# ucas-vg/PointTinyBenchmark

Hardware: NVIDIA H100
Metric: cpr_head_refine_img_per_s_1333x800 (higher is better)
Workload: dtype fp32

## Files before the change

pointtinybenchmark_b200/csrc/conv_tc.cu:

```cuda
#include "tc_ptx.cuh"
#include <cuda_bf16.h>
#include <stdlib.h>
#include <type_traits>

namespace ptb {

constexpr int CV_N = 256;
constexpr int CV_N_MAX = 512;
constexpr int CV_BM = 128;
constexpr int CV_NT = 128;
constexpr int CV_KB = 16;
constexpr int CV_KB_F16 = 32;
constexpr int CV_KH = 3;
constexpr int CV_A_STAGES = 4;
constexpr int CV_B_STAGES = 8;
constexpr uint32_t CV_A_BYTES = (CV_BM + 2 * 32) * 64;
constexpr uint32_t CV_B_BYTES = CV_NT * 64;
constexpr uint32_t CV_A_STAGE_BYTES = 2 * CV_A_BYTES;
constexpr uint32_t CV_B_STAGE_BYTES = 2 * CV_B_BYTES;
constexpr uint32_t CV_RING_BYTES = CV_A_STAGES * CV_A_STAGE_BYTES + CV_B_STAGES * CV_B_STAGE_BYTES;
constexpr uint32_t CV_SMEM_BYTES = CV_RING_BYTES + 1024  + 256 ;
static_assert(CV_SMEM_BYTES <= 227 * 1024, "the conv rings must fit the 227 KB of opt-in shared memory");
static_assert(2 * 8 * (CV_A_STAGES + CV_B_STAGES) + 8 <= 256, "the conv barriers and the item counter must fit their 256 B");
constexpr int CV_THREADS = 384;

struct ConvShape {
  int B, H, W, Cin;
  int tiles_h, tiles_w;
  int n_main, n_right, n_bottom, per_img, n_tiles;
  int right_w0, right_h;
  int bottom_h0;
  int n_slices;
  int taps;
  int n_out;
  int ldy;
};

struct ConvMaps {
  CUtensorMap x[3][2];
  CUtensorMap w[2];
};
struct TileAt {
  int b, h0, w0, shape, twl;
};
__device__ __forceinline__ TileAt tile_at(const ConvShape& cs, int tile) {
  TileAt t;
  t.b = tile / cs.per_img;
  const int r = tile - t.b * cs.per_img;
  if (r < cs.n_main) {
    t.shape = 0; t.twl = 4; t.h0 = (r / cs.tiles_w) * 8; t.w0 = (r % cs.tiles_w) * 16;
  } else if (r < cs.n_main + cs.n_right) {
    t.shape = 2; t.twl = 3; t.h0 = (r - cs.n_main) * 16; t.w0 = cs.right_w0;
  } else {
    t.shape = 1; t.twl = 5; t.h0 = cs.bottom_h0; t.w0 = (r - cs.n_main - cs.n_right) * 32;
  }
  return t;
}

constexpr int CV_GN_NONE = 0, CV_GN_F16 = 1, CV_GN_F32 = 2;
constexpr int CV_APPLY_WARPS = 3;
constexpr int CV_MMA_WARPS = 8;
struct GnFuse {
  const float* gamma;
  const float* beta;
  float eps;
  void* out;
  __half* out_l;
  int* overflow_flag;
  int* done;
};
constexpr uint32_t CV_CNT_OFFSET = 2 * 8 * (CV_A_STAGES + CV_B_STAGES);

__device__ __forceinline__ int ld_acquire_gpu(const int* p) {
  int v;
  asm volatile("ld.acquire.gpu.global.b32 %0, [%1];" : "=r"(v) : "l"(p) : "memory");
  return v;
}
__device__ __forceinline__ void red_release_gpu_add(int* p, int v) {
  asm volatile("red.release.gpu.global.add.s32 [%0], %1;" ::"l"(p), "r"(v) : "memory");
}
__device__ __forceinline__ int ld_acquire_cta_shared(uint32_t a) {
  int v;
  asm volatile("ld.acquire.cta.shared::cta.b32 %0, [%1];" : "=r"(v) : "r"(a) : "memory");
  return v;
}
__device__ __forceinline__ void red_release_cta_shared_add(uint32_t a, int v) {
  asm volatile("red.release.cta.shared::cta.add.s32 [%0], %1;" ::"r"(a), "r"(v) : "memory");
}
__device__ __forceinline__ void wait_count(const int* p, int target, int lane) {
  if (lane == 0) {
    uint32_t ns = 32, polls = 0;
    while (ld_acquire_gpu(p) < target) {
      __nanosleep(ns);
      if (ns < 1024) ns <<= 1;
      if (++polls > (1u << 24)) __trap();
    }
  }
  __syncwarp();
}
__device__ __forceinline__ void publish_image(uint32_t cnt, int* done_b, int item, int last, int lane) {
  if (lane == 0) {
    const int n = (last - item) / (int)gridDim.x + 1;
    const int through = (item - (int)blockIdx.x) / (int)gridDim.x + n;
    uint32_t ns = 32, polls = 0;
    while (ld_acquire_cta_shared(cnt) < through * (CV_MMA_WARPS / 2) || ld_acquire_cta_shared(cnt + 4) < through * (CV_MMA_WARPS / 2)) {
      __nanosleep(ns);
      if (ns < 1024) ns <<= 1;
      if (++polls > (1u << 24)) __trap();
    }
    red_release_gpu_add(done_b, n * CV_MMA_WARPS);
  }
  __syncwarp();
}

template <int GN>
__device__ __forceinline__ void gn_apply_item(const ConvShape& cs, const GnFuse& gf, const float* __restrict__ y,
                                              const double* __restrict__ stats, int item, int member, int team, int lane,
                                              bool& clamped) {
  const int tile = item / cs.n_slices, n0 = (item - tile * cs.n_slices) * CV_NT;
  const TileAt ta = tile_at(cs, tile);
  const int c = n0 + 4 * lane, g = c >> 3;
  const int HW = cs.H * cs.W, cpg = CV_N / 32;
  const double inv_n = 1.0 / ((double)HW * cpg);
  const double s = __ldcg(stats + ((size_t)ta.b * 32 + g) * 2), ss = __ldcg(stats + ((size_t)ta.b * 32 + g) * 2 + 1);
  const double mean = s * inv_n;
  double var = ss * inv_n - mean * mean;
  var = var < 0.0 ? 0.0 : var;
  const float rstd = (float)(1.0 / sqrt(var + (double)gf.eps));
  const float mu = (float)mean;
  const float4 ga = __ldg(reinterpret_cast<const float4*>(gf.gamma + c)), be = __ldg(reinterpret_cast<const float4*>(gf.beta + c));
  const int h_end = ta.shape == 2 ? cs.right_h : cs.H;
  const int tw_mask = (1 << ta.twl) - 1;
  const size_t img = (size_t)ta.b * HW * CV_N + c;
  const float* __restrict__ yb = y + img;
  constexpr int U = 4;
  for (int p0 = member; p0 < CV_BM; p0 += U * team) {
    float4 v[U];
    int at[U];
#pragma unroll
    for (int u = 0; u < U; ++u) {
      const int p = p0 + u * team;
      const int h = ta.h0 + (p >> ta.twl), w = ta.w0 + (p & tw_mask);
      at[u] = p < CV_BM && h < h_end && w < cs.W ? (h * cs.W + w) * CV_N : -1;
      if (at[u] >= 0) v[u] = __ldcg(reinterpret_cast<const float4*>(yb + at[u]));
    }
#pragma unroll
    for (int u = 0; u < U; ++u) {
      if (at[u] < 0) continue;
      float o[4] = {v[u].x, v[u].y, v[u].z, v[u].w};
      o[0] = fmaf((o[0] - mu) * rstd, ga.x, be.x); o[1] = fmaf((o[1] - mu) * rstd, ga.y, be.y);
      o[2] = fmaf((o[2] - mu) * rstd, ga.z, be.z); o[3] = fmaf((o[3] - mu) * rstd, ga.w, be.w);
#pragma unroll
      for (int j = 0; j < 4; ++j) o[j] = fmaxf(o[j], 0.f);
      if constexpr (GN == CV_GN_F16) {
        __align__(8) __half h[4], l[4];
#pragma unroll
        for (int j = 0; j < 4; ++j) {
          if (fabsf(o[j]) > 60000.f) { o[j] = copysignf(60000.f, o[j]); clamped = true; }
          split_h2(o[j], h[j], l[j]);
        }
        *reinterpret_cast<uint2*>(reinterpret_cast<__half*>(gf.out) + img + at[u]) = *reinterpret_cast<uint2*>(h);
        *reinterpret_cast<uint2*>(gf.out_l + img + at[u]) = *reinterpret_cast<uint2*>(l);
      } else {
        *reinterpret_cast<float4*>(reinterpret_cast<float*>(gf.out) + img + at[u]) = make_float4(o[0], o[1], o[2], o[3]);
      }
    }
  }
}

template <bool F16, int NT, bool A_LO_ZERO = false, typename OutT = float, int GN = CV_GN_NONE>
__global__ void __launch_bounds__(CV_THREADS, 1)
conv_tc_kernel(const __grid_constant__ ConvMaps mp, ConvShape cs, OutT* __restrict__ y, double* __restrict__ stats ,
               float out_scale, const float* __restrict__ dev_out_scale, const float* __restrict__ bias, GnFuse gf) {
  static_assert(F16 || NT == 128, "the TF32 mode runs 128-channel slices");
  static_assert(F16 || (!A_LO_ZERO && std::is_same<OutT, float>::value), "half-precision inputs and outputs belong to the fp16 mode");
  static_assert(GN == CV_GN_NONE || (F16 && NT == 128 && std::is_same<OutT, float>::value), "the fused GroupNorm apply runs on fp32 y, NT 128");
  constexpr int KBC = F16 ? CV_KB_F16 : CV_KB;
  extern __shared__ uint8_t smem_raw[];
  const uint32_t smem_base = (smem_u32(smem_raw) + 1023u) & ~1023u;
  const uint32_t sA_base = smem_base, sB_base = smem_base + CV_A_STAGES * CV_A_STAGE_BYTES;
  const uint32_t bar_base = smem_base + CV_RING_BYTES;
  auto full_a = [&](int s) { return bar_base + 8u * s; };
  auto empty_a = [&](int s) { return bar_base + 8u * (CV_A_STAGES + s); };
  auto full_b = [&](int s) { return bar_base + 8u * (2 * CV_A_STAGES + s); };
  auto empty_b = [&](int s) { return bar_base + 8u * (2 * CV_A_STAGES + CV_B_STAGES + s); };

  const int wg = threadIdx.x >> 7;
  const int kblocks_per_tap = cs.Cin / KBC;
  const int n_kh = cs.taps == 9 ? CV_KH : 1;
  const int n_boxes_item = (cs.taps / n_kh) * kblocks_per_tap;
  const int n_items = cs.n_tiles * cs.n_slices;

  if (threadIdx.x == 0) {
    for (int s = 0; s < CV_A_STAGES; ++s) {
      mbar_init(full_a(s), 1);
      mbar_init(empty_a(s), 8);
    }
    for (int s = 0; s < CV_B_STAGES; ++s) {
      mbar_init(full_b(s), 1);
      mbar_init(empty_b(s), 8);
    }
    if constexpr (GN != CV_GN_NONE) asm volatile("st.shared.v2.u32 [%0], {0, 0};" ::"r"(bar_base + CV_CNT_OFFSET) : "memory");
    asm volatile("fence.mbarrier_init.release.cluster;" ::: "memory");
  }
  __syncthreads();

  if (wg == 0) {
    if constexpr (GN != CV_GN_NONE) {
      regs_dealloc<72>();
      const int warp = threadIdx.x >> 5, lane = threadIdx.x & 31;
      if (warp >= 1) {
        const int items_per_img = cs.per_img * cs.n_slices;
        bool clamped = false;
        for (int item = blockIdx.x; item < n_items; item += gridDim.x) {
          const int b = item / items_per_img;
          if (b == cs.B - 1) break;
          if (warp == 1 && item - (int)gridDim.x < b * items_per_img)
            publish_image(bar_base + CV_CNT_OFFSET, gf.done + b, item, (b + 1) * items_per_img - 1, lane);
          wait_count(gf.done + b, items_per_img * CV_MMA_WARPS, lane);
          gn_apply_item<GN>(cs, gf, y, stats, item, warp - 1, CV_APPLY_WARPS, lane, clamped);
        }
        if (clamped && gf.overflow_flag) *gf.overflow_flag = 1;
      }
    } else {
      regs_dealloc<40>();
    }
    if (threadIdx.x == 0) {
      int a_st = 0, b_st = 0;
      uint32_t a_ph = 0, b_ph = 0;
      for (int item = blockIdx.x; item < n_items; item += gridDim.x) {
        const int tile = item / cs.n_slices, n0 = (item - tile * cs.n_slices) * NT;
        const TileAt ta = tile_at(cs, tile);
        const uint32_t a_bytes = (uint32_t)(CV_BM + ((n_kh - 1) << ta.twl)) * 64u;
        for (int ks = 0; ks < n_boxes_item; ++ks) {
          const int kw = cs.taps == 9 ? ks / kblocks_per_tap : 1, cblk = ks - (ks / kblocks_per_tap) * kblocks_per_tap;
          mbar_wait(empty_a(a_st), a_ph ^ 1u);
          const uint32_t sA_hi = sA_base + a_st * CV_A_STAGE_BYTES;
          mbar_expect_tx(full_a(a_st), (A_LO_ZERO ? 1 : 2) * a_bytes);
          const int aw = ta.w0 + kw - 1, ah = ta.h0 - (n_kh > 1 ? 1 : 0);
          tma_load_4d(&mp.x[ta.shape][0], full_a(a_st), sA_hi, cblk * KBC, aw, ah, ta.b);
          if constexpr (!A_LO_ZERO) tma_load_4d(&mp.x[ta.shape][1], full_a(a_st), sA_hi + CV_A_BYTES, cblk * KBC, aw, ah, ta.b);
          if (++a_st == CV_A_STAGES) { a_st = 0; a_ph ^= 1u; }
          for (int kh = 0; kh < n_kh; ++kh) {
            const int tap = cs.taps == 9 ? 3 * kh + kw : 0;
            const int kcol = tap * cs.Cin + cblk * KBC;
            mbar_wait(empty_b(b_st), b_ph ^ 1u);
            const uint32_t sB_hi = sB_base + b_st * CV_B_STAGE_BYTES;
            mbar_expect_tx(full_b(b_st), 2 * NT * 64);
            tma_load_2d(&mp.w[0], full_b(b_st), sB_hi, kcol, n0);
            tma_load_2d(&mp.w[1], full_b(b_st), sB_hi + CV_B_BYTES, kcol, n0);
            if (++b_st == CV_B_STAGES) { b_st = 0; b_ph ^= 1u; }
          }
        }
      }
    }
  } else {
    if constexpr (GN != CV_GN_NONE) regs_alloc<216>();
    else regs_alloc<232>();
    const int cw = wg - 1;
    const int t = threadIdx.x & 127, warp = t >> 5, lane = t & 31;
    const float sc = F16 ? (dev_out_scale ? __fmul_rn(out_scale, *dev_out_scale) : out_scale) : 1.f;
    float acc[NT / 2], cor[NT / 2];
    int a_st = 0, b_st = 0;
    uint32_t a_ph = 0, b_ph = 0;
    for (int item = blockIdx.x; item < n_items; item += gridDim.x) {
      const int tile = item / cs.n_slices, n0 = (item - tile * cs.n_slices) * NT;
      const TileAt ta = tile_at(cs, tile);
      const uint32_t kh_step = 64u << ta.twl;
      auto k_loop = [&](auto kh_n_) {
        constexpr int KH_N = decltype(kh_n_)::value;
        int prev_a = 0, prev_b = 0;
        for (int ks = 0; ks < n_boxes_item; ++ks) {
          mbar_wait(full_a(a_st), a_ph);
          const uint32_t sA_hi = sA_base + a_st * CV_A_STAGE_BYTES + (uint32_t)cw * (CV_BM * 64 / 2);
          const uint32_t sA_lo = sA_hi + CV_A_BYTES;
#pragma unroll
          for (int kh = 0; kh < KH_N; ++kh) {
            mbar_wait(full_b(b_st), b_ph);
            const uint32_t a_off = kh_step * kh, sB_hi = sB_base + b_st * CV_B_STAGE_BYTES, sB_lo = sB_hi + CV_B_BYTES;
            wgmma_fence();
#pragma unroll
            for (int k = 0; k < 2; ++k) {
              const uint64_t a_hi = gmma_desc(sA_hi + a_off + 32u * k, 16u, 512u, GMMA_SW64);
              const uint64_t a_lo = gmma_desc(sA_lo + a_off + 32u * k, 16u, 512u, GMMA_SW64);
              const uint64_t b_hi = gmma_desc(sB_hi + 32u * k, 16u, 512u, GMMA_SW64), b_lo = gmma_desc(sB_lo + 32u * k, 16u, 512u, GMMA_SW64);
              const uint32_t first = (ks | kh | k) != 0;
              if constexpr (F16) {
                wgmma_f16<0, 0>(acc, a_hi, b_hi, first);
                if constexpr (A_LO_ZERO) {
                  wgmma_f16<0, 0>(cor, a_hi, b_lo, first);
                } else {
                  wgmma_f16<0, 0>(cor, a_lo, b_hi, first);
                  wgmma_f16<0, 0>(cor, a_hi, b_lo, 1u);
                }
              } else {
                wgmma_tf32(acc, a_hi, b_hi, first);
                wgmma_tf32(cor, a_lo, b_hi, first);
                wgmma_tf32(cor, a_hi, b_lo, 1u);
              }
            }
            wgmma_commit();
            if ((ks | kh) != 0) {
              wgmma_wait<1>();
              if (lane == 0) {
                mbar_arrive(empty_b(prev_b));
                if (kh == 0) mbar_arrive(empty_a(prev_a));
              }
            }
            prev_b = b_st;
            if (++b_st == CV_B_STAGES) { b_st = 0; b_ph ^= 1u; }
          }
          prev_a = a_st;
          if (++a_st == CV_A_STAGES) { a_st = 0; a_ph ^= 1u; }
        }
        wgmma_wait<0>();
        if (lane == 0) { mbar_arrive(empty_b(prev_b)); mbar_arrive(empty_a(prev_a)); }
      };
      if (n_kh == CV_KH) k_loop(std::integral_constant<int, CV_KH>{});
      else k_loop(std::integral_constant<int, 1>{});

      const int h_end = ta.shape == 2 ? cs.right_h : cs.H;
      OutT* row_ptr[2];
      bool valid[2];
#pragma unroll
      for (int j = 0; j < 2; ++j) {
        const int r = 64 * cw + 16 * warp + (lane >> 2) + 8 * j;
        const int h = ta.h0 + (r >> ta.twl), w = ta.w0 + (r & ((1 << ta.twl) - 1));
        valid[j] = h < h_end && w < cs.W;
        row_ptr[j] = y + (((size_t)ta.b * cs.H + h) * cs.W + w) * cs.ldy;
      }
      float part[NT == 128 ? 32 : 1];
#pragma unroll
      for (int i = 0; i < NT / 8; ++i) {
        const int col = n0 + 8 * i + 2 * (lane & 3);
        float s = 0.f, ss = 0.f;
#pragma unroll
        for (int j = 0; j < 2; ++j) {
          float v0 = __fadd_rn(acc[4 * i + 2 * j], cor[4 * i + 2 * j]);
          float v1 = __fadd_rn(acc[4 * i + 2 * j + 1], cor[4 * i + 2 * j + 1]);
          if (F16) { v0 = __fmul_rn(v0, sc); v1 = __fmul_rn(v1, sc); }
          if (bias) {
            if (col < cs.n_out) v0 = v0 + __ldg(bias + col);
            if (col + 1 < cs.n_out) v1 = v1 + __ldg(bias + col + 1);
          }
          if (valid[j]) {
            if constexpr (std::is_same<OutT, float>::value) {
              if (col + 1 < cs.n_out) *reinterpret_cast<float2*>(row_ptr[j] + col) = make_float2(v0, v1);
              else if (col < cs.n_out) row_ptr[j][col] = v0;
            } else if constexpr (std::is_same<OutT, __half>::value) {
              if (col + 1 < cs.n_out) *reinterpret_cast<__half2*>(row_ptr[j] + col) = __halves2half2(__float2half_rn(v0), __float2half_rn(v1));
              else if (col < cs.n_out) row_ptr[j][col] = __float2half_rn(v0);
            } else {
              if (col + 1 < cs.n_out) *reinterpret_cast<__nv_bfloat162*>(row_ptr[j] + col) = __halves2bfloat162(__float2bfloat16_rn(v0), __float2bfloat16_rn(v1));
              else if (col < cs.n_out) row_ptr[j][col] = __float2bfloat16_rn(v0);
            }
            s += v0 + v1;
            ss = fmaf(v0, v0, ss);
            ss = fmaf(v1, v1, ss);
          }
        }
        if constexpr (NT == 128) { part[2 * i] = s; part[2 * i + 1] = ss; }
      }
      if constexpr (NT == 128) {
        if (stats) {
          auto level = [&](auto o_) {
            constexpr int o = decltype(o_)::value;
            const bool up = (lane & o) != 0;
#pragma unroll
            for (int i = 0; i < o; ++i) {
              const float send = up ? part[i] : part[i + o];
              const float recv = __shfl_xor_sync(0xffffffffu, send, o);
              part[i] = (up ? part[i + o] : part[i]) + recv;
            }
          };
          level(std::integral_constant<int, 16>{}); level(std::integral_constant<int, 8>{}); level(std::integral_constant<int, 4>{});
          level(std::integral_constant<int, 2>{}); level(std::integral_constant<int, 1>{});
          atomicAdd(stats + ((size_t)ta.b * 32 + (n0 >> 3) + (lane >> 1)) * 2 + (lane & 1), (double)part[0]);
        }
      }
      if constexpr (GN != CV_GN_NONE) {
        __syncwarp();
        if (lane == 0) red_release_cta_shared_add(bar_base + CV_CNT_OFFSET + 4u * cw, 1);
      }
    }
  }
  if constexpr (GN != CV_GN_NONE) {
    const int warp = threadIdx.x >> 5, lane = threadIdx.x & 31;
    if (warp >= 1) {
      const int items_per_img = cs.per_img * cs.n_slices, last0 = (cs.B - 1) * items_per_img;
      bool clamped = false;
      int item = (int)blockIdx.x;
      if (item < last0) item += (last0 - item + (int)gridDim.x - 1) / (int)gridDim.x * (int)gridDim.x;
      if (warp == 1 && item < n_items) publish_image(bar_base + CV_CNT_OFFSET, gf.done + cs.B - 1, item, n_items - 1, lane);
      for (; item < n_items; item += gridDim.x) {
        wait_count(gf.done + cs.B - 1, items_per_img * CV_MMA_WARPS, lane);
        gn_apply_item<GN>(cs, gf, y, stats, item, warp - 1, CV_APPLY_WARPS + CV_MMA_WARPS, lane, clamped);
      }
      if (clamped && gf.overflow_flag) *gf.overflow_flag = 1;
    }
  }
}

__device__ __forceinline__ float tf32_hi(float x) { return __uint_as_float(__float_as_uint(x) & 0xFFFFE000u); }

__global__ void __launch_bounds__(256)
split_tf32_kernel(const float4* __restrict__ x, long long n4, float4* __restrict__ hi, float4* __restrict__ lo) {
  for (long long i = (long long)blockIdx.x * 256 + threadIdx.x; i < n4; i += (long long)gridDim.x * 256) {
    const float4 v = __ldcs(x + i);
    float4 h = make_float4(tf32_hi(v.x), tf32_hi(v.y), tf32_hi(v.z), tf32_hi(v.w));
    hi[i] = h;
    lo[i] = make_float4(v.x - h.x, v.y - h.y, v.z - h.z, v.w - h.w);
  }
}

__global__ void __launch_bounds__(256)
gn_relu_apply_kernel(const float4* __restrict__ y, const double* __restrict__ stats, const float* __restrict__ gamma,
                     const float* __restrict__ beta, int HW, int C, int groups, float eps, int relu, long long n4,
                     float4* __restrict__ out_hi, float4* __restrict__ out_lo) {
  const int c4n = C >> 2;
  const int cpg = C / groups;
  const double inv_n = 1.0 / ((double)HW * cpg);
  for (long long i = (long long)blockIdx.x * 256 + threadIdx.x; i < n4; i += (long long)gridDim.x * 256) {
    const int c = (int)(i % c4n) * 4;
    const long long pix = i / c4n;
    const int b = (int)(pix / HW);
    const int g = c / cpg;
    const double s = stats[((size_t)b * groups + g) * 2], ss = stats[((size_t)b * groups + g) * 2 + 1];
    const double mean = s * inv_n;
    double var = ss * inv_n - mean * mean;
    var = var < 0.0 ? 0.0 : var;
    const float rstd = (float)(1.0 / sqrt(var + (double)eps));
    const float mu = (float)mean;
    const float4 v = __ldcs(y + i);
    const float4 ga = *reinterpret_cast<const float4*>(gamma + c), be = *reinterpret_cast<const float4*>(beta + c);
    float4 o;
    o.x = fmaf((v.x - mu) * rstd, ga.x, be.x);
    o.y = fmaf((v.y - mu) * rstd, ga.y, be.y);
    o.z = fmaf((v.z - mu) * rstd, ga.z, be.z);
    o.w = fmaf((v.w - mu) * rstd, ga.w, be.w);
    if (relu) { o.x = fmaxf(o.x, 0.f); o.y = fmaxf(o.y, 0.f); o.z = fmaxf(o.z, 0.f); o.w = fmaxf(o.w, 0.f); }
    if (out_lo) {
      const float4 h = make_float4(tf32_hi(o.x), tf32_hi(o.y), tf32_hi(o.z), tf32_hi(o.w));
      out_hi[i] = h;
      out_lo[i] = make_float4(o.x - h.x, o.y - h.y, o.z - h.z, o.w - h.w);
    } else {
      out_hi[i] = o;
    }
  }
}

__device__ __forceinline__ float pow2_scale_for(float amax) {
  if (!(amax > 0.f) || !isfinite(amax)) return 1.f;
  int e;
  frexpf(amax, &e);
  return ldexpf(1.f, 12 - e);
}

__device__ __forceinline__ float amax4(float m, const float4 v) {
  return fmaxf(m, fmaxf(fmaxf(fabsf(v.x), fabsf(v.y)), fmaxf(fabsf(v.z), fabsf(v.w))));
}

__global__ void __launch_bounds__(256) amax_abs_kernel(const float4* __restrict__ x, long long n4, unsigned int* __restrict__ out_bits) {
  float m = 0.f;
  const long long step = (long long)gridDim.x * 256;
  long long i = (long long)blockIdx.x * 256 + threadIdx.x;
  for (; i + 3 * step < n4; i += 4 * step) {
    const float4 v0 = x[i], v1 = x[i + step], v2 = x[i + 2 * step], v3 = x[i + 3 * step];
    m = amax4(amax4(amax4(amax4(m, v0), v1), v2), v3);
  }
  for (; i < n4; i += step) m = amax4(m, x[i]);
  m = warp_max(m);
  if ((threadIdx.x & 31) == 0) atomicMax(out_bits, __float_as_uint(m));
}

__device__ __forceinline__ void split8(const float4 a, const float4 b, float scale, uint4& ph, uint4& pl) {
  __align__(16) __half h[8], l[8];
  split_h2(a.x * scale, h[0], l[0]); split_h2(a.y * scale, h[1], l[1]);
  split_h2(a.z * scale, h[2], l[2]); split_h2(a.w * scale, h[3], l[3]);
  split_h2(b.x * scale, h[4], l[4]); split_h2(b.y * scale, h[5], l[5]);
  split_h2(b.z * scale, h[6], l[6]); split_h2(b.w * scale, h[7], l[7]);
  ph = *reinterpret_cast<uint4*>(h);
  pl = *reinterpret_cast<uint4*>(l);
}

__global__ void __launch_bounds__(256)
split_f16_kernel(const float4* __restrict__ x, long long n4, const unsigned int* __restrict__ dev_amax_bits,
                 uint2* __restrict__ hi, uint2* __restrict__ lo, float* __restrict__ inv_scale_out) {
  const float scale = dev_amax_bits ? pow2_scale_for(__uint_as_float(*dev_amax_bits)) : 1.f;
  if (inv_scale_out && blockIdx.x == 0 && threadIdx.x == 0) *inv_scale_out = 1.f / scale;
  const long long n8 = n4 >> 1;
  const long long step = (long long)gridDim.x * 256;
  uint4* hi8 = reinterpret_cast<uint4*>(hi);
  uint4* lo8 = reinterpret_cast<uint4*>(lo);
  const bool al16 = ((reinterpret_cast<uintptr_t>(hi) | reinterpret_cast<uintptr_t>(lo)) & 15) == 0;
  long long i = (long long)blockIdx.x * 256 + threadIdx.x;
  if (al16) {
    for (; i + step < n8; i += 2 * step) {
      const float4 a0 = __ldcs(x + 2 * i), a1 = __ldcs(x + 2 * i + 1);
      const float4 b0 = __ldcs(x + 2 * (i + step)), b1 = __ldcs(x + 2 * (i + step) + 1);
      uint4 ph, pl;
      split8(a0, a1, scale, ph, pl);
      hi8[i] = ph; lo8[i] = pl;
      split8(b0, b1, scale, ph, pl);
      hi8[i + step] = ph; lo8[i + step] = pl;
    }
    for (; i < n8; i += step) {
      uint4 ph, pl;
      split8(__ldcs(x + 2 * i), __ldcs(x + 2 * i + 1), scale, ph, pl);
      hi8[i] = ph; lo8[i] = pl;
    }
    i = 2 * n8 + (long long)blockIdx.x * 256 + threadIdx.x;
  }
  for (; i < n4; i += step) {
    const float4 v = __ldcs(x + i);
    __half h[4], l[4];
    split_h2(v.x * scale, h[0], l[0]); split_h2(v.y * scale, h[1], l[1]);
    split_h2(v.z * scale, h[2], l[2]); split_h2(v.w * scale, h[3], l[3]);
    hi[i] = *reinterpret_cast<uint2*>(h);
    lo[i] = *reinterpret_cast<uint2*>(l);
  }
}

__device__ __forceinline__ void bf16x8_to_f32(const uint4 v, float4& a, float4& b) {
  a = make_float4(__uint_as_float(v.x << 16), __uint_as_float(v.x & 0xFFFF0000u), __uint_as_float(v.y << 16), __uint_as_float(v.y & 0xFFFF0000u));
  b = make_float4(__uint_as_float(v.z << 16), __uint_as_float(v.z & 0xFFFF0000u), __uint_as_float(v.w << 16), __uint_as_float(v.w & 0xFFFF0000u));
}

__global__ void __launch_bounds__(256) amax_abs_bf16_kernel(const uint4* __restrict__ x, long long n8, unsigned int* __restrict__ out_bits) {
  float m = 0.f;
  const long long step = (long long)gridDim.x * 256;
  long long i = (long long)blockIdx.x * 256 + threadIdx.x;
  float4 a, b;
  for (; i + 3 * step < n8; i += 4 * step) {
    const uint4 v0 = x[i], v1 = x[i + step], v2 = x[i + 2 * step], v3 = x[i + 3 * step];
    bf16x8_to_f32(v0, a, b); m = amax4(amax4(m, a), b);
    bf16x8_to_f32(v1, a, b); m = amax4(amax4(m, a), b);
    bf16x8_to_f32(v2, a, b); m = amax4(amax4(m, a), b);
    bf16x8_to_f32(v3, a, b); m = amax4(amax4(m, a), b);
  }
  for (; i < n8; i += step) { bf16x8_to_f32(x[i], a, b); m = amax4(amax4(m, a), b); }
  m = warp_max(m);
  if ((threadIdx.x & 31) == 0) atomicMax(out_bits, __float_as_uint(m));
}

__global__ void __launch_bounds__(256)
split_f16_from_bf16_kernel(const uint4* __restrict__ x, long long n8, const unsigned int* __restrict__ dev_amax_bits,
                           uint4* __restrict__ hi, uint4* __restrict__ lo, float* __restrict__ inv_scale_out) {
  const float scale = pow2_scale_for(__uint_as_float(*dev_amax_bits));
  if (blockIdx.x == 0 && threadIdx.x == 0) *inv_scale_out = 1.f / scale;
  const long long step = (long long)gridDim.x * 256;
  long long i = (long long)blockIdx.x * 256 + threadIdx.x;
  float4 a, b;
  uint4 ph, pl;
  for (; i + step < n8; i += 2 * step) {
    const uint4 v0 = __ldcs(x + i), v1 = __ldcs(x + i + step);
    bf16x8_to_f32(v0, a, b); split8(a, b, scale, ph, pl);
    hi[i] = ph; lo[i] = pl;
    bf16x8_to_f32(v1, a, b); split8(a, b, scale, ph, pl);
    hi[i + step] = ph; lo[i + step] = pl;
  }
  for (; i < n8; i += step) {
    bf16x8_to_f32(__ldcs(x + i), a, b); split8(a, b, scale, ph, pl);
    hi[i] = ph; lo[i] = pl;
  }
}

__global__ void __launch_bounds__(256)
gn_relu_apply_f16_kernel(const float4* __restrict__ y, const double* __restrict__ stats, const float* __restrict__ gamma,
                         const float* __restrict__ beta, int HW, int C, int groups, float eps, int relu, long long n4,
                         uint2* __restrict__ out_h, uint2* __restrict__ out_l, int* __restrict__ overflow_flag) {
  const int c4n = C >> 2;
  const int cpg = C / groups;
  const double inv_n = 1.0 / ((double)HW * cpg);
  for (long long i = (long long)blockIdx.x * 256 + threadIdx.x; i < n4; i += (long long)gridDim.x * 256) {
    const int c = (int)(i % c4n) * 4;
    const long long pix = i / c4n;
    const int b = (int)(pix / HW);
    const int g = c / cpg;
    const double s = stats[((size_t)b * groups + g) * 2], ss = stats[((size_t)b * groups + g) * 2 + 1];
    const double mean = s * inv_n;
    double var = ss * inv_n - mean * mean;
    var = var < 0.0 ? 0.0 : var;
    const float rstd = (float)(1.0 / sqrt(var + (double)eps));
    const float mu = (float)mean;
    const float4 v = __ldcs(y + i);
    const float4 ga = *reinterpret_cast<const float4*>(gamma + c), be = *reinterpret_cast<const float4*>(beta + c);
    float o[4];
    o[0] = fmaf((v.x - mu) * rstd, ga.x, be.x); o[1] = fmaf((v.y - mu) * rstd, ga.y, be.y);
    o[2] = fmaf((v.z - mu) * rstd, ga.z, be.z); o[3] = fmaf((v.w - mu) * rstd, ga.w, be.w);
    __half h[4], l[4];
#pragma unroll
    for (int j = 0; j < 4; ++j) {
      if (relu) o[j] = fmaxf(o[j], 0.f);
      if (fabsf(o[j]) > 60000.f) { o[j] = copysignf(60000.f, o[j]); if (overflow_flag) *overflow_flag = 1; }
      split_h2(o[j], h[j], l[j]);
    }
    out_h[i] = *reinterpret_cast<uint2*>(h);
    out_l[i] = *reinterpret_cast<uint2*>(l);
  }
}

__global__ void __launch_bounds__(256)
gn_relu_apply_f16_v8_kernel(const float4* __restrict__ y, const double* __restrict__ stats, const float* __restrict__ gamma,
                            const float* __restrict__ beta, int HW, int C, int groups, float eps, int relu, int pix_per_cta,
                            uint4* __restrict__ out_h, uint4* __restrict__ out_l, int* __restrict__ overflow_flag) {
  const int tpp = C >> 3;
  const int ppp = 256 / tpp;
  const int c = (threadIdx.x % tpp) * 8;
  const int b = blockIdx.y;
  const int cpg = C / groups;
  const int g = c / cpg;
  const double inv_n = 1.0 / ((double)HW * cpg);
  const double s = stats[((size_t)b * groups + g) * 2], ss = stats[((size_t)b * groups + g) * 2 + 1];
  const double mean = s * inv_n;
  double var = ss * inv_n - mean * mean;
  var = var < 0.0 ? 0.0 : var;
  const float rstd = (float)(1.0 / sqrt(var + (double)eps));
// ... 460 lines not shown
```

pointtinybenchmark_b200/csrc/tc_ptx.cuh:

```cuda
#pragma once
#include "ptb_common.cuh"
#include <cuda.h>
#include <cuda_fp16.h>

namespace ptb {

__device__ __forceinline__ uint32_t smem_u32(const void* p) { return (uint32_t)__cvta_generic_to_shared(p); }

__device__ __forceinline__ void mbar_init(uint32_t bar, uint32_t count) {
  asm volatile("mbarrier.init.shared::cta.b64 [%0], %1;" ::"r"(bar), "r"(count) : "memory");
}
__device__ __forceinline__ void mbar_expect_tx(uint32_t bar, uint32_t bytes) {
  asm volatile("mbarrier.arrive.expect_tx.shared::cta.b64 _, [%0], %1;" ::"r"(bar), "r"(bytes) : "memory");
}
__device__ __forceinline__ void mbar_arrive(uint32_t bar) {
  asm volatile("mbarrier.arrive.shared::cta.b64 _, [%0];" ::"r"(bar) : "memory");
}
__device__ __forceinline__ bool mbar_try_wait(uint32_t bar, uint32_t parity) {
  uint32_t ok;
  asm volatile(
      "{\n\t.reg .pred p;\n\t"
      "mbarrier.try_wait.parity.shared::cta.b64 p, [%1], %2;\n\t"
      "selp.u32 %0, 1, 0, p;\n\t}"
      : "=r"(ok)
      : "r"(bar), "r"(parity)
      : "memory");
  return ok != 0;
}
__device__ __forceinline__ void mbar_wait(uint32_t bar, uint32_t parity) {
  uint32_t spins = 0;
  while (!mbar_try_wait(bar, parity)) {
    if (++spins > (1u << 28)) __trap();
  }
}
__device__ __forceinline__ void tma_load_4d(const CUtensorMap* tm, uint32_t bar, uint32_t dst, int c0, int c1, int c2, int c3) {
  asm volatile(
      "cp.async.bulk.tensor.4d.shared::cluster.global.mbarrier::complete_tx::bytes [%0], [%1, {%3, %4, %5, %6}], [%2];"
      ::"r"(dst), "l"(tm), "r"(bar), "r"(c0), "r"(c1), "r"(c2), "r"(c3)
      : "memory");
}
__device__ __forceinline__ void tma_load_2d(const CUtensorMap* tm, uint32_t bar, uint32_t dst, int c0, int c1) {
  asm volatile(
      "cp.async.bulk.tensor.2d.shared::cluster.global.mbarrier::complete_tx::bytes [%0], [%1, {%3, %4}], [%2];"
      ::"r"(dst), "l"(tm), "r"(bar), "r"(c0), "r"(c1)
      : "memory");
}
__device__ __forceinline__ void fence_async_smem() { asm volatile("fence.proxy.async.shared::cta;" ::: "memory"); }

constexpr uint32_t GMMA_SW128 = 1, GMMA_SW64 = 2;
__device__ __forceinline__ uint64_t gmma_desc(uint32_t smem_addr, uint32_t lbo, uint32_t sbo, uint32_t layout) {
  uint64_t d = 0;
  d |= (uint64_t)((smem_addr & 0x3FFFF) >> 4);
  d |= (uint64_t)((lbo >> 4) & 0x3FFF) << 16;
  d |= (uint64_t)((sbo >> 4) & 0x3FFF) << 32;
  d |= (uint64_t)layout << 62;
  return d;
}
__device__ __forceinline__ void wgmma_fence() { asm volatile("wgmma.fence.sync.aligned;" ::: "memory"); }
__device__ __forceinline__ void wgmma_commit() { asm volatile("wgmma.commit_group.sync.aligned;" ::: "memory"); }
template <int N>
__device__ __forceinline__ void wgmma_wait() { asm volatile("wgmma.wait_group.sync.aligned %0;" ::"n"(N) : "memory"); }
template <int R>
__device__ __forceinline__ void regs_dealloc() { asm volatile("setmaxnreg.dec.sync.aligned.u32 %0;" ::"n"(R)); }
template <int R>
__device__ __forceinline__ void regs_alloc() { asm volatile("setmaxnreg.inc.sync.aligned.u32 %0;" ::"n"(R)); }
template <int TA, int TB>
__device__ __forceinline__ void wgmma_f16(float (&d)[64], uint64_t da, uint64_t db, uint32_t scale_d) {
  asm volatile(
      "{\n\t.reg .pred p;\n\t"
      "setp.ne.b32 p, %66, 0;\n\t"
      "wgmma.mma_async.sync.aligned.m64n128k16.f32.f16.f16 "
      "{%0, %1, %2, %3, %4, %5, %6, %7, %8, %9, %10, %11, %12, %13, %14, %15,"
      " %16, %17, %18, %19, %20, %21, %22, %23, %24, %25, %26, %27, %28, %29, %30, %31,"
      " %32, %33, %34, %35, %36, %37, %38, %39, %40, %41, %42, %43, %44, %45, %46, %47,"
      " %48, %49, %50, %51, %52, %53, %54, %55, %56, %57, %58, %59, %60, %61, %62, %63}, "
      "%64, %65, p, 1, 1, %67, %68;\n\t}"
      : "+f"(d[0]), "+f"(d[1]), "+f"(d[2]), "+f"(d[3]), "+f"(d[4]), "+f"(d[5]), "+f"(d[6]), "+f"(d[7]),
        "+f"(d[8]), "+f"(d[9]), "+f"(d[10]), "+f"(d[11]), "+f"(d[12]), "+f"(d[13]), "+f"(d[14]), "+f"(d[15]),
        "+f"(d[16]), "+f"(d[17]), "+f"(d[18]), "+f"(d[19]), "+f"(d[20]), "+f"(d[21]), "+f"(d[22]), "+f"(d[23]),
        "+f"(d[24]), "+f"(d[25]), "+f"(d[26]), "+f"(d[27]), "+f"(d[28]), "+f"(d[29]), "+f"(d[30]), "+f"(d[31]),
        "+f"(d[32]), "+f"(d[33]), "+f"(d[34]), "+f"(d[35]), "+f"(d[36]), "+f"(d[37]), "+f"(d[38]), "+f"(d[39]),
        "+f"(d[40]), "+f"(d[41]), "+f"(d[42]), "+f"(d[43]), "+f"(d[44]), "+f"(d[45]), "+f"(d[46]), "+f"(d[47]),
        "+f"(d[48]), "+f"(d[49]), "+f"(d[50]), "+f"(d[51]), "+f"(d[52]), "+f"(d[53]), "+f"(d[54]), "+f"(d[55]),
        "+f"(d[56]), "+f"(d[57]), "+f"(d[58]), "+f"(d[59]), "+f"(d[60]), "+f"(d[61]), "+f"(d[62]), "+f"(d[63])
      : "l"(da), "l"(db), "r"(scale_d), "n"(TA), "n"(TB));
}

template <int TA, int TB>
__device__ __forceinline__ void wgmma_f16(float (&d)[32], uint64_t da, uint64_t db, uint32_t scale_d) {
  asm volatile(
      "{\n\t.reg .pred p;\n\t"
      "setp.ne.b32 p, %34, 0;\n\t"
      "wgmma.mma_async.sync.aligned.m64n64k16.f32.f16.f16 "
      "{%0, %1, %2, %3, %4, %5, %6, %7, %8, %9, %10, %11, %12, %13, %14, %15,"
      " %16, %17, %18, %19, %20, %21, %22, %23, %24, %25, %26, %27, %28, %29, %30, %31}, "
      "%32, %33, p, 1, 1, %35, %36;\n\t}"
      : "+f"(d[0]), "+f"(d[1]), "+f"(d[2]), "+f"(d[3]), "+f"(d[4]), "+f"(d[5]), "+f"(d[6]), "+f"(d[7]),
        "+f"(d[8]), "+f"(d[9]), "+f"(d[10]), "+f"(d[11]), "+f"(d[12]), "+f"(d[13]), "+f"(d[14]), "+f"(d[15]),
        "+f"(d[16]), "+f"(d[17]), "+f"(d[18]), "+f"(d[19]), "+f"(d[20]), "+f"(d[21]), "+f"(d[22]), "+f"(d[23]),
        "+f"(d[24]), "+f"(d[25]), "+f"(d[26]), "+f"(d[27]), "+f"(d[28]), "+f"(d[29]), "+f"(d[30]), "+f"(d[31])
      : "l"(da), "l"(db), "r"(scale_d), "n"(TA), "n"(TB));
}

template <int TA, int TB>
__device__ __forceinline__ void wgmma_f16(float (&d)[16], uint64_t da, uint64_t db, uint32_t scale_d) {
  asm volatile(
      "{\n\t.reg .pred p;\n\t"
      "setp.ne.b32 p, %18, 0;\n\t"
      "wgmma.mma_async.sync.aligned.m64n32k16.f32.f16.f16 "
      "{%0, %1, %2, %3, %4, %5, %6, %7, %8, %9, %10, %11, %12, %13, %14, %15}, "
      "%16, %17, p, 1, 1, %19, %20;\n\t}"
      : "+f"(d[0]), "+f"(d[1]), "+f"(d[2]), "+f"(d[3]), "+f"(d[4]), "+f"(d[5]), "+f"(d[6]), "+f"(d[7]),
        "+f"(d[8]), "+f"(d[9]), "+f"(d[10]), "+f"(d[11]), "+f"(d[12]), "+f"(d[13]), "+f"(d[14]), "+f"(d[15])
      : "l"(da), "l"(db), "r"(scale_d), "n"(TA), "n"(TB));
}

template <int TA, int TB>
__device__ __forceinline__ void wgmma_f16(float (&d)[8], uint64_t da, uint64_t db, uint32_t scale_d) {
  asm volatile(
      "{\n\t.reg .pred p;\n\t"
      "setp.ne.b32 p, %10, 0;\n\t"
      "wgmma.mma_async.sync.aligned.m64n16k16.f32.f16.f16 "
      "{%0, %1, %2, %3, %4, %5, %6, %7}, "
      "%8, %9, p, 1, 1, %11, %12;\n\t}"
      : "+f"(d[0]), "+f"(d[1]), "+f"(d[2]), "+f"(d[3]), "+f"(d[4]), "+f"(d[5]), "+f"(d[6]), "+f"(d[7])
      : "l"(da), "l"(db), "r"(scale_d), "n"(TA), "n"(TB));
}

__device__ __forceinline__ void wgmma_tf32(float (&d)[64], uint64_t da, uint64_t db, uint32_t scale_d) {
  asm volatile(
      "{\n\t.reg .pred p;\n\t"
      "setp.ne.b32 p, %66, 0;\n\t"
      "wgmma.mma_async.sync.aligned.m64n128k8.f32.tf32.tf32 "
      "{%0, %1, %2, %3, %4, %5, %6, %7, %8, %9, %10, %11, %12, %13, %14, %15,"
      " %16, %17, %18, %19, %20, %21, %22, %23, %24, %25, %26, %27, %28, %29, %30, %31,"
      " %32, %33, %34, %35, %36, %37, %38, %39, %40, %41, %42, %43, %44, %45, %46, %47,"
      " %48, %49, %50, %51, %52, %53, %54, %55, %56, %57, %58, %59, %60, %61, %62, %63}, "
      "%64, %65, p, 1, 1;\n\t}"
      : "+f"(d[0]), "+f"(d[1]), "+f"(d[2]), "+f"(d[3]), "+f"(d[4]), "+f"(d[5]), "+f"(d[6]), "+f"(d[7]),
        "+f"(d[8]), "+f"(d[9]), "+f"(d[10]), "+f"(d[11]), "+f"(d[12]), "+f"(d[13]), "+f"(d[14]), "+f"(d[15]),
        "+f"(d[16]), "+f"(d[17]), "+f"(d[18]), "+f"(d[19]), "+f"(d[20]), "+f"(d[21]), "+f"(d[22]), "+f"(d[23]),
        "+f"(d[24]), "+f"(d[25]), "+f"(d[26]), "+f"(d[27]), "+f"(d[28]), "+f"(d[29]), "+f"(d[30]), "+f"(d[31]),
        "+f"(d[32]), "+f"(d[33]), "+f"(d[34]), "+f"(d[35]), "+f"(d[36]), "+f"(d[37]), "+f"(d[38]), "+f"(d[39]),
        "+f"(d[40]), "+f"(d[41]), "+f"(d[42]), "+f"(d[43]), "+f"(d[44]), "+f"(d[45]), "+f"(d[46]), "+f"(d[47]),
        "+f"(d[48]), "+f"(d[49]), "+f"(d[50]), "+f"(d[51]), "+f"(d[52]), "+f"(d[53]), "+f"(d[54]), "+f"(d[55]),
        "+f"(d[56]), "+f"(d[57]), "+f"(d[58]), "+f"(d[59]), "+f"(d[60]), "+f"(d[61]), "+f"(d[62]), "+f"(d[63])
      : "l"(da), "l"(db), "r"(scale_d));
}


__device__ __forceinline__ void split_h2(float v, __half& h, __half& l) {
  h = __float2half_rn(v);
  l = __float2half_rn(v - __half2float(h));
}

typedef CUresult (*EncodeTiledFn)(CUtensorMap*, CUtensorMapDataType, cuuint32_t, void*, const cuuint64_t*, const cuuint64_t*,
                                  const cuuint32_t*, const cuuint32_t*, CUtensorMapInterleave, CUtensorMapSwizzle,
                                  CUtensorMapL2promotion, CUtensorMapFloatOOBfill);
EncodeTiledFn tc_get_encode();

}
```

Baseline: 2405.

## Feed f16 conv wgmma A-hi operand from registers via ldmatrix

In the f16 path, the high half of the A tile is now loaded into registers with ldmatrix and used by register-sourced wgmma (RS form). Previously it was read from shared memory through a descriptor for each of the two or three MMAs that use it. The register fragments are double-buffered across kh/box iterations, and the box loop is unrolled by two so the buffer index stays compile-time. The aim is to cut repeated shared-memory operand traffic for A. The cost is extra register pressure in an already heavy consumer warpgroup, plus dependence on the swizzle address math being correct.

```diff
diff --git a/pointtinybenchmark_b200/csrc/conv_tc.cu b/pointtinybenchmark_b200/csrc/conv_tc.cu
--- a/pointtinybenchmark_b200/csrc/conv_tc.cu
+++ b/pointtinybenchmark_b200/csrc/conv_tc.cu
@@ -263,6 +263,9 @@
     float acc[NT / 2], cor[NT / 2];
     int a_st = 0, b_st = 0;
     uint32_t a_ph = 0, b_ph = 0;
+    const int a_row = 16 * warp + (lane & 15);
+    const uint32_t a_lane[2] = {(uint32_t)(a_row * 64 + (((0 + (lane >> 4)) ^ ((a_row >> 1) & 3)) << 4)),
+                                (uint32_t)(a_row * 64 + (((2 + (lane >> 4)) ^ ((a_row >> 1) & 3)) << 4))};
     for (int item = blockIdx.x; item < n_items; item += gridDim.x) {
       const int tile = item / cs.n_slices, n0 = (item - tile * cs.n_slices) * NT;
       const TileAt ta = tile_at(cs, tile);
@@ -270,30 +273,38 @@
       auto k_loop = [&](auto kh_n_) {
         constexpr int KH_N = decltype(kh_n_)::value;
         int prev_a = 0, prev_b = 0;
-        for (int ks = 0; ks < n_boxes_item; ++ks) {
+        [[maybe_unused]] uint32_t ahi[2][2][4];
+        auto box = [&](int ks, auto p_) {
+          constexpr int P = decltype(p_)::value;
           mbar_wait(full_a(a_st), a_ph);
           const uint32_t sA_hi = sA_base + a_st * CV_A_STAGE_BYTES + (uint32_t)cw * (CV_BM * 64 / 2);
           const uint32_t sA_lo = sA_hi + CV_A_BYTES;
 #pragma unroll
           for (int kh = 0; kh < KH_N; ++kh) {
+            [[maybe_unused]] const int q = (P * KH_N + kh) & 1;
+            const uint32_t a_off = kh_step * kh;
+            if constexpr (F16) {
+              ldmatrix_x4(ahi[q][0], sA_hi + a_off + a_lane[0]);
+              ldmatrix_x4(ahi[q][1], sA_hi + a_off + a_lane[1]);
+            }
             mbar_wait(full_b(b_st), b_ph);
-            const uint32_t a_off = kh_step * kh, sB_hi = sB_base + b_st * CV_B_STAGE_BYTES, sB_lo = sB_hi + CV_B_BYTES;
+            const uint32_t sB_hi = sB_base + b_st * CV_B_STAGE_BYTES, sB_lo = sB_hi + CV_B_BYTES;
             wgmma_fence();
 #pragma unroll
             for (int k = 0; k < 2; ++k) {
-              const uint64_t a_hi = gmma_desc(sA_hi + a_off + 32u * k, 16u, 512u, GMMA_SW64);
               const uint64_t a_lo = gmma_desc(sA_lo + a_off + 32u * k, 16u, 512u, GMMA_SW64);
               const uint64_t b_hi = gmma_desc(sB_hi + 32u * k, 16u, 512u, GMMA_SW64), b_lo = gmma_desc(sB_lo + 32u * k, 16u, 512u, GMMA_SW64);
               const uint32_t first = (ks | kh | k) != 0;
               if constexpr (F16) {
-                wgmma_f16<0, 0>(acc, a_hi, b_hi, first);
+                wgmma_f16_rs(acc, ahi[q][k], b_hi, first);
                 if constexpr (A_LO_ZERO) {
-                  wgmma_f16<0, 0>(cor, a_hi, b_lo, first);
+                  wgmma_f16_rs(cor, ahi[q][k], b_lo, first);
                 } else {
                   wgmma_f16<0, 0>(cor, a_lo, b_hi, first);
-                  wgmma_f16<0, 0>(cor, a_hi, b_lo, 1u);
+                  wgmma_f16_rs(cor, ahi[q][k], b_lo, 1u);
                 }
               } else {
+                const uint64_t a_hi = gmma_desc(sA_hi + a_off + 32u * k, 16u, 512u, GMMA_SW64);
                 wgmma_tf32(acc, a_hi, b_hi, first);
                 wgmma_tf32(cor, a_lo, b_hi, first);
                 wgmma_tf32(cor, a_hi, b_lo, 1u);
@@ -312,7 +323,15 @@
           }
           prev_a = a_st;
           if (++a_st == CV_A_STAGES) { a_st = 0; a_ph ^= 1u; }
+        };
+        int ks = 0;
+        if constexpr (F16) {
+          for (; ks + 1 < n_boxes_item; ks += 2) {
+            box(ks, std::integral_constant<int, 0>{});
+            box(ks + 1, std::integral_constant<int, 1>{});
+          }
         }
+        for (; ks < n_boxes_item; ++ks) box(ks, std::integral_constant<int, 0>{});
         wgmma_wait<0>();
         if (lane == 0) { mbar_arrive(empty_b(prev_b)); mbar_arrive(empty_a(prev_a)); }
       };
diff --git a/pointtinybenchmark_b200/csrc/tc_ptx.cuh b/pointtinybenchmark_b200/csrc/tc_ptx.cuh
--- a/pointtinybenchmark_b200/csrc/tc_ptx.cuh
+++ b/pointtinybenchmark_b200/csrc/tc_ptx.cuh
@@ -127,6 +127,72 @@
       : "l"(da), "l"(db), "r"(scale_d), "n"(TA), "n"(TB));
 }
 
+__device__ __forceinline__ void wgmma_f16_rs(float (&d)[64], const uint32_t (&a)[4], uint64_t db, uint32_t scale_d) {
+  asm volatile(
+      "{\n\t.reg .pred p;\n\t"
+      "setp.ne.b32 p, %69, 0;\n\t"
+      "wgmma.mma_async.sync.aligned.m64n128k16.f32.f16.f16 "
+      "{%0, %1, %2, %3, %4, %5, %6, %7, %8, %9, %10, %11, %12, %13, %14, %15,"
+      " %16, %17, %18, %19, %20, %21, %22, %23, %24, %25, %26, %27, %28, %29, %30, %31,"
+      " %32, %33, %34, %35, %36, %37, %38, %39, %40, %41, %42, %43, %44, %45, %46, %47,"
+      " %48, %49, %50, %51, %52, %53, %54, %55, %56, %57, %58, %59, %60, %61, %62, %63}, "
+      "{%64, %65, %66, %67}, %68, p, 1, 1, 0;\n\t}"
+      : "+f"(d[0]), "+f"(d[1]), "+f"(d[2]), "+f"(d[3]), "+f"(d[4]), "+f"(d[5]), "+f"(d[6]), "+f"(d[7]),
+        "+f"(d[8]), "+f"(d[9]), "+f"(d[10]), "+f"(d[11]), "+f"(d[12]), "+f"(d[13]), "+f"(d[14]), "+f"(d[15]),
+        "+f"(d[16]), "+f"(d[17]), "+f"(d[18]), "+f"(d[19]), "+f"(d[20]), "+f"(d[21]), "+f"(d[22]), "+f"(d[23]),
+        "+f"(d[24]), "+f"(d[25]), "+f"(d[26]), "+f"(d[27]), "+f"(d[28]), "+f"(d[29]), "+f"(d[30]), "+f"(d[31]),
+        "+f"(d[32]), "+f"(d[33]), "+f"(d[34]), "+f"(d[35]), "+f"(d[36]), "+f"(d[37]), "+f"(d[38]), "+f"(d[39]),
+        "+f"(d[40]), "+f"(d[41]), "+f"(d[42]), "+f"(d[43]), "+f"(d[44]), "+f"(d[45]), "+f"(d[46]), "+f"(d[47]),
+        "+f"(d[48]), "+f"(d[49]), "+f"(d[50]), "+f"(d[51]), "+f"(d[52]), "+f"(d[53]), "+f"(d[54]), "+f"(d[55]),
+        "+f"(d[56]), "+f"(d[57]), "+f"(d[58]), "+f"(d[59]), "+f"(d[60]), "+f"(d[61]), "+f"(d[62]), "+f"(d[63])
+      : "r"(a[0]), "r"(a[1]), "r"(a[2]), "r"(a[3]), "l"(db), "r"(scale_d));
+}
+
+__device__ __forceinline__ void wgmma_f16_rs(float (&d)[32], const uint32_t (&a)[4], uint64_t db, uint32_t scale_d) {
+  asm volatile(
+      "{\n\t.reg .pred p;\n\t"
+      "setp.ne.b32 p, %37, 0;\n\t"
+      "wgmma.mma_async.sync.aligned.m64n64k16.f32.f16.f16 "
+      "{%0, %1, %2, %3, %4, %5, %6, %7, %8, %9, %10, %11, %12, %13, %14, %15,"
+      " %16, %17, %18, %19, %20, %21, %22, %23, %24, %25, %26, %27, %28, %29, %30, %31}, "
+      "{%32, %33, %34, %35}, %36, p, 1, 1, 0;\n\t}"
+      : "+f"(d[0]), "+f"(d[1]), "+f"(d[2]), "+f"(d[3]), "+f"(d[4]), "+f"(d[5]), "+f"(d[6]), "+f"(d[7]),
+        "+f"(d[8]), "+f"(d[9]), "+f"(d[10]), "+f"(d[11]), "+f"(d[12]), "+f"(d[13]), "+f"(d[14]), "+f"(d[15]),
+        "+f"(d[16]), "+f"(d[17]), "+f"(d[18]), "+f"(d[19]), "+f"(d[20]), "+f"(d[21]), "+f"(d[22]), "+f"(d[23]),
+        "+f"(d[24]), "+f"(d[25]), "+f"(d[26]), "+f"(d[27]), "+f"(d[28]), "+f"(d[29]), "+f"(d[30]), "+f"(d[31])
+      : "r"(a[0]), "r"(a[1]), "r"(a[2]), "r"(a[3]), "l"(db), "r"(scale_d));
+}
+
+__device__ __forceinline__ void wgmma_f16_rs(float (&d)[16], const uint32_t (&a)[4], uint64_t db, uint32_t scale_d) {
+  asm volatile(
+      "{\n\t.reg .pred p;\n\t"
+      "setp.ne.b32 p, %21, 0;\n\t"
+      "wgmma.mma_async.sync.aligned.m64n32k16.f32.f16.f16 "
+      "{%0, %1, %2, %3, %4, %5, %6, %7, %8, %9, %10, %11, %12, %13, %14, %15}, "
+      "{%16, %17, %18, %19}, %20, p, 1, 1, 0;\n\t}"
+      : "+f"(d[0]), "+f"(d[1]), "+f"(d[2]), "+f"(d[3]), "+f"(d[4]), "+f"(d[5]), "+f"(d[6]), "+f"(d[7]),
+        "+f"(d[8]), "+f"(d[9]), "+f"(d[10]), "+f"(d[11]), "+f"(d[12]), "+f"(d[13]), "+f"(d[14]), "+f"(d[15])
+      : "r"(a[0]), "r"(a[1]), "r"(a[2]), "r"(a[3]), "l"(db), "r"(scale_d));
+}
+
+__device__ __forceinline__ void wgmma_f16_rs(float (&d)[8], const uint32_t (&a)[4], uint64_t db, uint32_t scale_d) {
+  asm volatile(
+      "{\n\t.reg .pred p;\n\t"
+      "setp.ne.b32 p, %13, 0;\n\t"
+      "wgmma.mma_async.sync.aligned.m64n16k16.f32.f16.f16 "
+      "{%0, %1, %2, %3, %4, %5, %6, %7}, "
+      "{%8, %9, %10, %11}, %12, p, 1, 1, 0;\n\t}"
+      : "+f"(d[0]), "+f"(d[1]), "+f"(d[2]), "+f"(d[3]), "+f"(d[4]), "+f"(d[5]), "+f"(d[6]), "+f"(d[7])
+      : "r"(a[0]), "r"(a[1]), "r"(a[2]), "r"(a[3]), "l"(db), "r"(scale_d));
+}
+
+__device__ __forceinline__ void ldmatrix_x4(uint32_t (&r)[4], uint32_t addr) {
+  asm volatile("ldmatrix.sync.aligned.m8n8.x4.shared.b16 {%0, %1, %2, %3}, [%4];"
+               : "=r"(r[0]), "=r"(r[1]), "=r"(r[2]), "=r"(r[3])
+               : "r"(addr)
+               : "memory");
+}
+
 __device__ __forceinline__ void wgmma_tf32(float (&d)[64], uint64_t da, uint64_t db, uint32_t scale_d) {
   asm volatile(
       "{\n\t.reg .pred p;\n\t"
```

Result: slower. 2363, median of 6 (-1.7%).
